# wahn/rs_pbrt

Measured on NVIDIA H100. Metric: Mrays/s, higher is better.
Workload: dtype f32

## Files before the change

### rs_pbrt_b200/csrc/pb_kernels.cuh

```cuda
#pragma once
#include "pb_bsdf.cuh"
#include "pb_interaction.cuh"
#include "pb_sobol.cuh"
#include "pb_texture.cuh"
#include "pb_material.cuh"

namespace pb {

#define PB_TRACE_THREADS 128
#define PB_TRACE_SMEM_BYTES 49152
#define PB_SHADE_THREADS 128
#define PB_SMEM_SOBOL_BYTES 49152

#ifdef PB_HOST_EMU
PB_D void mbar_init(uint64_t*, uint32_t) {}
PB_D void mbar_fence_init() {}
PB_D void mbar_expect_tx(uint64_t*, uint32_t) {}
PB_D void tma_bulk_g2s(void* dst_smem, const void* src_gmem, uint32_t bytes, uint64_t*) { memcpy(dst_smem, src_gmem, bytes); }
PB_D void mbar_wait(uint64_t*, uint32_t) { __syncthreads(); }
#define PB_DYNAMIC_SMEM(name) unsigned char* name = emu::g_dyn_smem
#else
#define PB_DYNAMIC_SMEM(name) extern __shared__ __align__(16) unsigned char name[]
PB_D void mbar_fence_init() { asm volatile("fence.mbarrier_init.release.cluster;" ::: "memory"); }
PB_D uint32_t smem_u32(const void* p) { return (uint32_t)__cvta_generic_to_shared(p); }
// ... 315 lines not shown
    float4* o = wide + 4 * (size_t)i;
    o[0] = make_float4(a[0].x, a[0].y, a[0].z, a[0].w);
    o[1] = make_float4(b[0].x, b[0].y, a[1].x, a[1].y);
    o[2] = make_float4(a[1].z, a[1].w, b[1].x, b[1].y);
    o[3] = make_float4(__uint_as_float(ref[0]), __uint_as_float(ref[1]), __uint_as_float((meta >> 16) & 3u), 0.0f);
}
#ifndef PB_WIDE_MIN_BLOCKS
#define PB_WIDE_MIN_BLOCKS 0
#endif
#ifndef PB_WIDE_INST_MIN_BLOCKS
#define PB_WIDE_INST_MIN_BLOCKS 8
#endif
#if PB_WIDE_MIN_BLOCKS > 0
#define PB_WIDE_BOUNDS __launch_bounds__(PB_TRACE_THREADS, PB_WIDE_MIN_BLOCKS)
#else
#define PB_WIDE_BOUNDS __launch_bounds__(PB_TRACE_THREADS)
#endif
__global__ void PB_WIDE_BOUNDS k_trace_wide_plain(DScene sc, TraceIO io, const uint32_t* __restrict__ d_nrays, uint32_t* __restrict__ cursor, DCounters* cnt, int walk_steps) {
    trace_rays_wide<false>(sc, sc.wide, sc.tri_verts, io, *d_nrays, cursor, cnt, walk_steps);
}
__global__ void __launch_bounds__(PB_TRACE_THREADS, PB_WIDE_INST_MIN_BLOCKS) k_trace_wide_inst(DScene sc, TraceIO io, const uint32_t* __restrict__ d_nrays, uint32_t* __restrict__ cursor,
                                                                                             DCounters* cnt, int walk_steps) {
    trace_rays_wide<true>(sc, sc.wide, sc.tri_verts, io, *d_nrays, cursor, cnt, walk_steps);
}

__global__ void PB_WIDE_BOUNDS k_trace_wide_spec(DScene sc, TraceIO io, const uint32_t* __restrict__ d_nrays,
                                                                                        uint32_t* __restrict__ cursor, DCounters* cnt, int walk_steps) {
    trace_rays_wide_spec(sc, sc.wide, sc.tri_verts, io, *d_nrays, cursor, cnt, walk_steps);
}

__global__ void __launch_bounds__(256) k_rayprep(const float4* __restrict__ rays, const uint32_t* __restrict__ d_nrays, float4* __restrict__ pre) {
    const uint32_t n = *d_nrays;
    for (uint32_t i = blockIdx.x * blockDim.x + threadIdx.x; i < n; i += gridDim.x * blockDim.x) {
        const float4 a = rays[2 * (size_t)i], b = rays[2 * (size_t)i + 1];
        const RayPre r = make_ray(mk3(a.x, a.y, a.z), mk3(b.x, b.y, b.z));
        float4 p0, p1;
        pack_ray(r, p0, p1);
        pre[2 * (size_t)i] = p0;
        pre[2 * (size_t)i + 1] = p1;
    }
}

__global__ void __launch_bounds__(256) k_sort(DScene sc, DPaths ps, DLightGrid grid, uint32_t spatial, uint32_t instancing, const uint32_t* __restrict__ queue,
                                             const uint32_t* __restrict__ d_count, uint32_t* __restrict__ cls_queue, uint32_t cls_stride,
                                             uint32_t* __restrict__ cls_count, uint32_t* __restrict__ reset_count_out, uint32_t* __restrict__ reset_nrays) {
    if (blockIdx.x == 0 && threadIdx.x == 0) { *reset_count_out = 0u; *reset_nrays = 0u; }
    const uint32_t count = *d_count;
    const uint32_t lane = threadIdx.x & 31;
    const uint32_t total = (count + 31u) & ~31u;
    for (uint32_t qi = blockIdx.x * blockDim.x + threadIdx.x; qi < total; qi += gridDim.x * blockDim.x) {
        uint32_t cls = 0xffffffffu, slot = 0;
        if (qi < count) {
            slot = queue[qi];
            cls = 0;
            if (__float_as_uint(ps.L[slot].w) & PF_HAS_RAY) {
                float4 h = ps.hit[slot];
                int prim = __float_as_int(h.x);
                if (prim >= 0) {
                    float4 c = __ldg(sc.tri_verts + 3 * (size_t)prim + 2);
                    uint32_t mat = __float_as_uint(c.y);
                    const uint32_t inst = sc.n_instances ? ps.hit_inst[slot] : 0xffffffffu;
                    const bool moved = inst != 0xffffffffu && !sc.instances[inst].identity;
                    if (moved && instancing == 0u) mat = 0xffffffffu;
                    cls = (mat == 0xffffffffu) ? 1u : ((uint32_t)sc.materials[mat].cls & 0xffu);
                    if (spatial) {
                        float4 a = __ldg(sc.tri_verts + 3 * (size_t)prim), b = __ldg(sc.tri_verts + 3 * (size_t)prim + 1);
                        V3 p = mk3(a.x, a.y, a.z) * h.y + mk3(a.w, b.x, b.y) * h.z + mk3(b.z, b.w, c.x) * h.w;
                        if (moved) {
                            const float* m = sc.instances[inst].m;
                            const float xp = m[0] * p.x + m[1] * p.y + m[2] * p.z + m[3], yp = m[4] * p.x + m[5] * p.y + m[6] * p.z + m[7];
                            const float zp = m[8] * p.x + m[9] * p.y + m[10] * p.z + m[11], wp = m[12] * p.x + m[13] * p.y + m[14] * p.z + m[15];
                            p = mk3(xp, yp, zp);
                            if (wp != 1.0f) { const float inv = 1.0f / wp; p = mk3(inv * xp, inv * yp, inv * zp); }
                        }
                        uint32_t v = light_voxel(sc, grid, p);
                        if (grid.state[v] == 0 && atomicCAS(&grid.state[v], 0, 1) == 0) {
                            if (grid.row) {
                                uint32_t r = atomicAdd(grid.n_request + 1, 1u);
                                if (r >= grid.max_rows) { r = 0u; atomicOr(grid.n_request + 2, 1u); }
                                grid.row[v] = (int)r;
                            }
                            grid.request[atomicAdd(grid.n_request, 1u)] = v;
                        }
                    }
                }
            }
        }
        unsigned peers = __match_any_sync(0xffffffffu, cls);
        uint32_t base = 0;
        int leader = __ffs(peers) - 1;
        if (cls != 0xffffffffu && (int)lane == leader) base = atomicAdd(cls_count + cls, (uint32_t)__popc(peers));
        base = __shfl_sync(0xffffffffu, base, leader);
        if (cls != 0xffffffffu) cls_queue[(size_t)cls * cls_stride + base + (uint32_t)__popc(peers & ((1u << lane) - 1u))] = slot;
    }
}

__global__ void k_lightgrid_contrib(DScene sc, DLightGrid g, const float* __restrict__ halton ) {
    uint32_t nreq = *g.n_request;
    uint32_t total = nreq * (uint32_t)g.n_lights;
    for (uint32_t i = blockIdx.x * blockDim.x + threadIdx.x; i < total; i += gridDim.x * blockDim.x) {
        uint32_t v = g.request[i / (uint32_t)g.n_lights], j = i % (uint32_t)g.n_lights;
        int ix = (int)(v % (uint32_t)g.nv[0]), iy = (int)((v / (uint32_t)g.nv[0]) % (uint32_t)g.nv[1]), iz = (int)(v / ((uint32_t)g.nv[0] * (uint32_t)g.nv[1]));
        float t0x = (float)ix / (float)g.nv[0], t0y = (float)iy / (float)g.nv[1], t0z = (float)iz / (float)g.nv[2];
        float t1x = (float)(ix + 1) / (float)g.nv[0], t1y = (float)(iy + 1) / (float)g.nv[1], t1z = (float)(iz + 1) / (float)g.nv[2];
        V3 vmin = mk3(lerpf(t0x, sc.wb_min[0], sc.wb_max[0]), lerpf(t0y, sc.wb_min[1], sc.wb_max[1]), lerpf(t0z, sc.wb_min[2], sc.wb_max[2]));
        V3 vmax = mk3(lerpf(t1x, sc.wb_min[0], sc.wb_max[0]), lerpf(t1y, sc.wb_min[1], sc.wb_max[1]), lerpf(t1z, sc.wb_min[2], sc.wb_max[2]));
        const DLight& light = sc.lights[j];
        float contrib = 0.0f;
        for (int s = 0; s < 128; ++s) {
            const float* hs = halton + 5 * s;
            V3 po = mk3(lerpf(__ldg(hs), vmin.x, vmax.x), lerpf(__ldg(hs + 1), vmin.y, vmax.y), lerpf(__ldg(hs + 2), vmin.z, vmax.z));
            float pdf = 0.0f;
            V3 wi;
            LightSample ls;
            Sp li = light_sample_li<false>(sc, light, po, make_float2(__ldg(hs + 3), __ldg(hs + 4)), wi, pdf, ls);
            if (pdf > 0.0f) contrib += lum(li) / pdf;
        }
        g.contrib[g.row_of(v) * g.n_lights + j] = contrib;
    }
}
__global__ void k_lightgrid_build(DLightGrid g) {
    uint32_t nreq = *g.n_request;
    const int nl = g.n_lights;
    for (uint32_t i = blockIdx.x * blockDim.x + threadIdx.x; i < nreq; i += gridDim.x * blockDim.x) {
        uint32_t v = g.request[i];
        const size_t r = g.row_of(v);
        const float* c = g.contrib + r * nl;
        float sum = 0.0f;
        for (int j = 0; j < nl; ++j) sum += c[j];
        float avg = sum / (float)(128 * nl);
        float min_contrib = (avg > 0.0f) ? 0.001f * avg : 1.0f;
        float* func = g.func + r * nl;
        float* cdf = g.cdf + r * (nl + 1);
        cdf[0] = 0.0f;
        for (int j = 0; j < nl; ++j) {
            float f = fmaxf(c[j], min_contrib);
            func[j] = f;
            cdf[j + 1] = cdf[j] + f / (float)nl;
        }
// ... 219 lines not shown
    PB_DYNAMIC_SMEM(smem_raw);
    __shared__ __align__(8) uint64_t s_bar;
    if (blockIdx.x == 0 && threadIdx.x < PB_SHADE_CLASSES) {
        reset_cls_count[threadIdx.x] = 0u;
        if (threadIdx.x == 0) { *reset_cursor = 0u; if (reset_requests) *reset_requests = 0u; }
    }
    const uint32_t* tab = nib;
    const uint32_t tab_stride = sobol_cfg & 0xffffu;
    if (!HALTON && (sobol_cfg >> 31)) {
        const uint32_t bytes = n_chunks * 64u * tab_stride;
        if (threadIdx.x == 0) {
            mbar_init(&s_bar, 1);
            mbar_fence_init();
        }
        __syncthreads();
        if (threadIdx.x == 0) {
            mbar_expect_tx(&s_bar, bytes);
            for (uint32_t off = 0; off < bytes; off += 16384u)
                tma_bulk_g2s(smem_raw + off, reinterpret_cast<const unsigned char*>(nib) + off, min(16384u, bytes - off), &s_bar);
        }
        mbar_wait(&s_bar, 0);
        tab = reinterpret_cast<const uint32_t*>(smem_raw);
    }
    __shared__ uint32_t s_tiles[PB_SHADE_CLASSES + 1];
    if (threadIdx.x == 0) {
        uint32_t acc = 0;
        for (uint32_t c = 0; c < PB_SHADE_CLASSES; ++c) { s_tiles[c] = acc; if (c >= cls_lo && c < cls_hi) acc += (cls_count[c] + 31u) >> 5; }
        s_tiles[PB_SHADE_CLASSES] = acc;
    }
    __syncthreads();
    const uint32_t total_tiles = s_tiles[PB_SHADE_CLASSES];
    const int NONSPEC = BSDF_ALL & ~BSDF_SPECULAR;
    const float inf = __int_as_float(0x7f800000);
    uint32_t n_light_tests = 0, n_slots = 0, n_vertices = 0;
    const uint32_t warps_total = (gridDim.x * blockDim.x) >> 5;
    const uint32_t warp_id = (blockIdx.x * blockDim.x + threadIdx.x) >> 5;
    const uint32_t lane = threadIdx.x & 31;
    for (uint32_t tile = warp_id; tile < total_tiles; tile += warps_total) {
        uint32_t cls = 0;
        while (cls + 1 < PB_SHADE_CLASSES && tile >= s_tiles[cls + 1]) ++cls;
        const uint32_t qi = (tile - s_tiles[cls]) * 32u + lane;
        const uint32_t count = cls_count[cls];
        bool push = false, emit_ext = false, emit_sh = false, emit_mis = false;
        float4 ext0, ext1, sh0, sh1, mis0, mis1;
        ext0 = ext1 = sh0 = sh1 = mis0 = mis1 = make_float4(0.0f, 0.0f, 0.0f, 0.0f);
        uint32_t slot = 0;
        if (qi < count) {
            slot = cls_queue[(size_t)cls * cls_stride + qi];
            n_slots++;
            const float4 Lf = ps.L[slot];
            const float4 st_hit = ps.hit[slot], st_rd = ps.ray_d[slot], st_beta = ps.beta[slot];
            const uint2 st_sobol = ps.sobol[slot];
            const uint32_t st_dim = ps.dim[slot];
            const float4 st_ld = ps.ld_light[slot], st_mh = ps.mis_hit[slot], st_md = ps.mis_d[slot], st_mf = ps.mis_f[slot], st_nb = ps.nee_beta[slot];
            const uint32_t st_occl = ps.occl[slot];
            uint32_t flags = __float_as_uint(Lf.w);
            Sp L = mksp(Lf.x, Lf.y, Lf.z);
            if (flags & (PF_HAS_SHADOW | PF_HAS_MIS)) {
                Sp ld = sp1(0.0f);
                const float4 a = st_ld;
                if ((flags & PF_HAS_SHADOW) && st_occl == 0u) ld = ld + mksp(a.x, a.y, a.z);
                if (flags & PF_HAS_MIS) {
                    const float4 mh = st_mh;
                    int mprim = __float_as_int(mh.x);
                    if (mprim >= 0) {
                        const float4 md = st_md, mf = st_mf;
                        int light_num = (int)__float_as_uint(md.w);
                        V3 lp, ln;
                        int hit_light;
                        tri_point_normal(sc, (uint32_t)mprim, mh.y, mh.z, mh.w, lp, ln, hit_light);
                        if (hit_light == light_num) {
                            Sp le = light_L(sc.lights[light_num], ln, -mk3(md.x, md.y, md.z));
                            if (!is_black(le)) ld = ld + mksp(mf.x, mf.y, mf.z) * le * sp1(1.0f) * a.w / mf.w;
                        }
                    } else if (!AREA_ONLY && sc.n_inf) {
                        const float4 md = st_md, mf = st_mf;
                        Sp le = light_le(sc, sc.lights[__float_as_uint(md.w)], mk3(md.x, md.y, md.z));
                        if (!is_black(le)) ld = ld + mksp(mf.x, mf.y, mf.z) * le * sp1(1.0f) * a.w / mf.w;
                    }
                }
                const float4 nb = st_nb;
                L = L + mksp(nb.x, nb.y, nb.z) * spdiv0(ld, nb.w);
            }
            uint32_t out_flags = 0;
            if (!AREA_ONLY && cls == 0u && sc.n_inf && (flags & PF_HAS_RAY) && __float_as_int(st_hit.x) < 0) {
                if ((flags >> PF_BOUNCES_SHIFT) == 0 || (flags & PF_SPECULAR_BOUNCE)) {
                    const Sp beta = mksp(st_beta.x, st_beta.y, st_beta.z);
                    const V3 rd = mk3(st_rd.x, st_rd.y, st_rd.z);
                    for (uint32_t k = 0; k < sc.n_inf; ++k) L = L + beta * light_le(sc, sc.lights[sc.inf[k]], rd);
                }
            }
            if (cls != 0u) {
                uint32_t bounces = flags >> PF_BOUNCES_SHIFT;
                bool specular_bounce = (flags & PF_SPECULAR_BOUNCE) != 0;
                const float4 hit = st_hit;
                int prim = __float_as_int(hit.x);
                if (prim >= 0) {
                    n_vertices++;
                    const float4 rd4 = st_rd, b4 = st_beta;
                    V3 rd = mk3(rd4.x, rd4.y, rd4.z);
                    Sp beta = mksp(b4.x, b4.y, b4.z);
                    float eta_scale = b4.w;
                    V3 wo = -rd;
                    V3 wo_nee = wo;
                    Isect is = INST ? hit_interaction(sc, rp.instancing, (uint32_t)prim, hit.y, hit.z, hit.w, ps.hit_inst[slot], rd, wo_nee)
                                              : tri_interaction(sc, (uint32_t)prim, hit.y, hit.z, hit.w);
                    if (bounces == 0 || specular_bounce) {
                        const Sp le = is.area_light >= 0 ? light_L(sc.lights[is.area_light], is.n, wo) : sp1(0.0f);
                        L = L + beta * le;
                    }
                    if (bounces < rp.max_depth) {
                        if (is.material == 0xffffffffu) {
                            V3 o = offset_ray_origin(is.p, is.p_error, is.n, rd);
                            ext0 = make_float4(o.x, o.y, o.z, inf);
                            ext1 = make_float4(rd.x, rd.y, rd.z, __uint_as_float(slot | (RAY_EXTEND << 30)));
                            emit_ext = true;
                            out_flags = (flags & ~0xffu) | (flags & PF_SPECULAR_BOUNCE) | PF_HAS_RAY;
                        } else {
                            BsdfFrame B;
                            B.mat = sc.materials + is.material;
                            if (SPEC == 0 && (B.mat->cls & PB_MAT_TEXTURED)) {
                                if (B.mat->cls & PB_MAT_BUMPED) {
                                    const float4 f0 = ps.slot_frame[2 * (size_t)slot], f1 = ps.slot_frame[2 * (size_t)slot + 1];
                                    is.ns = mk3(f0.x, f0.y, f0.z);
                                    is.sh_dpdu = mk3(f1.x, f1.y, f1.z);
                                }
                                B.mat = ps.slot_mat + slot;
                            }
                            B.ns = is.ns;
                            B.ng = is.n;
                            B.ss = norm3(is.sh_dpdu);
                            B.ts = cross3(is.ns, B.ss);
                            const uint2 si = st_sobol;
                            SobolT sob;
                            sob.nib = tab;
                            sob.ds = tab_stride;
                            sob.n_chunks = n_chunks;
                            sob.index = ((uint64_t)si.y << 32) | si.x;
                            sob.dim = st_dim;
                            sob.overflow = false;
                            uint32_t nee_flags = 0;
                            if (SPEC >= 1 ? pb_spec_has_nonspecular(SPEC) : (B.mat->nonspecular > 0)) {
                                Sp ld_now = sp1(0.0f);
                                const int nl = grid.n_lights;
                                if (nl > 0) {
                                    const size_t v = (rp.light_strategy == 2u) ? grid.row_of(light_voxel(sc, grid, is.p)) : (size_t)0;
                                    float choice_pdf;
                                    float u5[5];
                                    if (HALTON) {
#pragma unroll
                                        for (int k = 0; k < 5; ++k) u5[k] = halton_scrambled(rp, (uint32_t)sob.index, min(sob.dim + (uint32_t)k, (uint32_t)(PB_HALTON_DIMS - 1)));
                                    } else sobolT_fill<5>(sob, u5);
                                    const float u_choice = sobolT_take<HALTON>(sob, 1) ? u5[0] : 0.0f;
                                    int light_num = sample_discrete(grid.func + v * nl, grid.cdf + v * (nl + 1), grid.func_int[v], nl,
                                                                    u_choice, choice_pdf);
                                    if (choice_pdf != 0.0f) {
                                        float2 u_light = make_float2(0.0f, 0.0f), u_scat = make_float2(0.0f, 0.0f);
                                        if (sobolT_take<HALTON>(sob, 2)) u_light = make_float2(u5[1], u5[2]);
                                        if (sobolT_take<HALTON>(sob, 2)) u_scat = make_float2(u5[3], u5[4]);
                                        const DLight& light = sc.lights[light_num];
                                        V3 wi = mk3(0.0f, 0.0f, 0.0f);
                                        float light_pdf = 0.0f, scattering_pdf = 0.0f, mis_w = 0.0f;
                                        Sp a = sp1(0.0f);
                                        LightSample ls;
                                        Sp li = light_sample_li<AREA_ONLY>(sc, light, is.p, u_light, wi, light_pdf, ls);
                                        if (light_pdf > 0.0f && !is_black(li)) {
                                            Sp f = bsdf_f<SPEC>(B, wo_nee, wi, NONSPEC) * sp1(absdot3(wi, is.ns));
                                            scattering_pdf = bsdf_pdf<SPEC>(B, wo_nee, wi, NONSPEC);
                                            if (!is_black(f)) {
                                                V3 origin = offset_ray_origin(is.p, is.p_error, is.n, ls.p - is.p);
                                                V3 target = offset_ray_origin(ls.p, ls.p_error, ls.n, origin - ls.p);
                                                V3 sd = target - origin;
                                                if (!AREA_ONLY && light_is_delta(light)) a = f * li / light_pdf;
                                                else {
                                                    float w = power_heuristic(light_pdf, scattering_pdf);
                                                    a = f * li * sp1(w) / light_pdf;
                                                }
                                                sh0 = make_float4(origin.x, origin.y, origin.z, 1.0f - PB_SHADOW_EPSILON);
                                                sh1 = make_float4(sd.x, sd.y, sd.z, __uint_as_float(slot | (RAY_SHADOW << 30)));
                                                emit_sh = true;
                                                nee_flags |= PF_HAS_SHADOW;
                                            }
                                        }
                                        int st = 0;
                                        Sp f2 = sp1(0.0f);
                                        if (AREA_ONLY || !light_is_delta(light)) {
                                            f2 = bsdf_sample_f<SPEC>(B, wo_nee, wi, u_scat, scattering_pdf, NONSPEC, st);
                                            f2 = f2 * sp1(absdot3(wi, is.ns));
                                        }
                                        if (!is_black(f2) && scattering_pdf > 0.0f) {
                                            V3 mo = offset_ray_origin(is.p, is.p_error, is.n, wi);
                                            if (AREA_ONLY || light.kind == 0u) n_light_tests++;
                                            float lp = light_pdf_li<AREA_ONLY>(sc, light, is.p, mo, wi);
                                            if (lp != 0.0f) {
                                                mis_w = power_heuristic(scattering_pdf, lp);
                                                mis0 = make_float4(mo.x, mo.y, mo.z, inf);
                                                mis1 = make_float4(wi.x, wi.y, wi.z, __uint_as_float(slot | (RAY_MIS << 30)));
                                                emit_mis = true;
                                                ps.mis_d[slot] = make_float4(wi.x, wi.y, wi.z, __uint_as_float((uint32_t)light_num));
                                                ps.mis_f[slot] = make_float4(f2.r, f2.g, f2.b, scattering_pdf);
                                                nee_flags |= PF_HAS_MIS;
                                            }
                                        }
                                        if (nee_flags) {
                                            ps.ld_light[slot] = make_float4(a.r, a.g, a.b, mis_w);
                                            ps.nee_beta[slot] = make_float4(beta.r, beta.g, beta.b, choice_pdf);
                                        } else ld_now = spdiv0(sp1(0.0f), choice_pdf);
                                    }
                                }
                                if (!nee_flags) L = L + beta * ld_now;
                            }
                            V3 wi = mk3(0.0f, 0.0f, 0.0f);
                            float pdf = 0.0f;
                            int st = 255;
                            float u3[3];
                            if (HALTON) {
                                u3[0] = halton_scrambled(rp, (uint32_t)sob.index, min(sob.dim, (uint32_t)(PB_HALTON_DIMS - 1)));
                                u3[1] = halton_scrambled(rp, (uint32_t)sob.index, min(sob.dim + 1u, (uint32_t)(PB_HALTON_DIMS - 1)));
                                u3[2] = 0.0f;
                            } else sobolT_fill<3>(sob, u3);
                            const float2 u_bsdf = sobolT_take<HALTON>(sob, 2) ? make_float2(u3[0], u3[1]) : make_float2(0.0f, 0.0f);
                            Sp f = bsdf_sample_f<SPEC>(B, wo, wi, u_bsdf, pdf, BSDF_ALL, st);
                            bool alive = !(is_black(f) || pdf == 0.0f);
                            if (alive) {
                                beta = beta * ((f * absdot3(wi, is.ns)) / pdf);
                                specular_bounce = (st & BSDF_SPECULAR) != 0;
                                if ((st & BSDF_SPECULAR) && (st & BSDF_TRANSMISSION)) {
                                    float eta = B.mat->eta;
                                    if (dot3(wo, is.n) > 0.0f) eta_scale *= eta * eta;
                                    else eta_scale *= 1.0f / (eta * eta);
                                }
                                V3 o = offset_ray_origin(is.p, is.p_error, is.n, wi);
                                Sp rr_beta = beta * eta_scale;
                                if (maxsp(rr_beta) < rp.rr_threshold && bounces > 3) {
                                    float q = fmaxf(0.05f, 1.0f - maxsp(rr_beta));
                                    if (HALTON) u3[2] = halton_scrambled(rp, (uint32_t)sob.index, min(sob.dim, (uint32_t)(PB_HALTON_DIMS - 1)));
                                    const float u_rr = sobolT_take<HALTON>(sob, 1) ? u3[2] : 0.0f;
                                    if (u_rr < q) alive = false;
                                    else beta = beta / (1.0f - q);
                                }
                                if (alive) {
                                    ext0 = make_float4(o.x, o.y, o.z, inf);
                                    ext1 = make_float4(wi.x, wi.y, wi.z, __uint_as_float(slot | (RAY_EXTEND << 30)));
                                    emit_ext = true;
                                    ps.ray_d[slot] = make_float4(wi.x, wi.y, wi.z, 0.0f);
                                    ps.beta[slot] = make_float4(beta.r, beta.g, beta.b, eta_scale);
                                    ps.dim[slot] = sob.dim;
                                    out_flags = ((bounces + 1) << PF_BOUNCES_SHIFT) | (specular_bounce ? PF_SPECULAR_BOUNCE : 0u) | PF_HAS_RAY;
                                }
                            }
                            out_flags |= nee_flags;
                            if (sob.overflow) atomicOr(d_error, 1u);
                        }
                    }
                }
            }
            ps.L[slot] = make_float4(L.r, L.g, L.b, __uint_as_float(out_flags));
            push = (out_flags & (PF_HAS_RAY | PF_HAS_SHADOW | PF_HAS_MIS)) != 0;
        }
        const unsigned mp = __ballot_sync(0xffffffffu, push);
        const unsigned me = __ballot_sync(0xffffffffu, emit_ext), mm = __ballot_sync(0xffffffffu, emit_mis), ms = __ballot_sync(0xffffffffu, emit_sh);
        const uint32_t ne = (uint32_t)__popc(me), nm = (uint32_t)__popc(mm), nsh = (uint32_t)__popc(ms);
        uint32_t qbase = 0, rbase = 0;
        if (lane == 0) {
            if (mp) qbase = atomicAdd(d_count_out, (uint32_t)__popc(mp));
            if (ne + nm + nsh) rbase = atomicAdd(d_nrays, ne + nm + nsh);
        }
        qbase = __shfl_sync(0xffffffffu, qbase, 0);
        rbase = __shfl_sync(0xffffffffu, rbase, 0);
        if (push) queue_out[qbase + (uint32_t)__popc(mp & ((1u << lane) - 1u))] = slot;
        const unsigned lt = (1u << lane) - 1u;
        if (emit_ext) { size_t q = rbase + (uint32_t)__popc(me & lt); rays[2 * q] = ext0; rays[2 * q + 1] = ext1; if (ray_keys) ray_keys[q] = ray_key(sc, ext0, ext1) & key_mask; }
        if (emit_mis) { size_t q = rbase + ne + (uint32_t)__popc(mm & lt); rays[2 * q] = mis0; rays[2 * q + 1] = mis1; if (ray_keys) ray_keys[q] = ray_key(sc, mis0, mis1) & key_mask; }
        if (emit_sh) { size_t q = rbase + ne + nm + (uint32_t)__popc(ms & lt); rays[2 * q] = sh0; rays[2 * q + 1] = sh1; if (ray_keys) ray_keys[q] = ray_key(sc, sh0, sh1) & key_mask; }
    }
    uint32_t t = warp_sum(n_light_tests);
    if (lane == 0 && t) atomicAdd(&cnt->light_tri_tests, (unsigned long long)t);
    t = warp_sum(n_slots);
    if (lane == 0 && t) atomicAdd(&cnt->shade_slots, (unsigned long long)t);
    t = warp_sum(n_vertices);
    if (lane == 0 && t) atomicAdd(&cnt->shaded_vertices, (unsigned long long)t);
}

PB_D V3 uniform_sample_hemisphere(float2 u) {
    float z = u.x;
    float r = sqrtf(fmaxf(0.0f, 1.0f - z * z));
    float phi = 2.0f * PB_PI * u.y;
    float sp, cp;
    sincos_rn(phi, sp, cp);
    return mk3(r * cp, r * sp, z);
}
__global__ void __launch_bounds__(256) k_ao_shade(DScene sc, DRender rp, DPaths ps, BatchInfo bi, uint32_t ao_n, uint32_t ao_cos, const uint32_t* __restrict__ nib,
                                                  uint32_t n_chunks, const uint64_t* __restrict__ vdc, const uint64_t* __restrict__ vdci,
                                                  float4* __restrict__ rays, float* __restrict__ weight, uint32_t* __restrict__ d_nrays) {
    __shared__ uint64_t s_vdc[52], s_vdci[52];
    if (threadIdx.x < 52) {
        uint32_t m = rp.log2_res;
        s_vdc[threadIdx.x] = m ? vdc[(m - 1) * 52 + threadIdx.x] : 0;
        s_vdci[threadIdx.x] = m ? vdci[(m - 1) * 52 + threadIdx.x] : 0;
    }
    __syncthreads();
    const uint32_t n_paths = bi.n_pixels * bi.n_samples;
    const uint64_t total = (uint64_t)n_paths * ao_n;
    const uint64_t gid = (uint64_t)blockIdx.x * blockDim.x + threadIdx.x;
    float4 r0 = make_float4(0.0f, 0.0f, 0.0f, 0.0f), r1 = r0;
    bool live = false;
    if (gid < total) {
// ... 141 lines not shown
```

### rs_pbrt_b200/csrc/pbrt_gpu.cu

```cuda
#include <sched.h>

#include <algorithm>
#include <chrono>
#include <cmath>
#include <cstdio>
#include <cstdlib>
#include <atomic>
#include <cstring>
#include <functional>
#include <map>
#include <memory>
#include <mutex>
#include <string>
#include <thread>
#include <vector>

#include "../../include/pbrt_gpu.h"
#include "pb_kernels.cuh"
#include "pb_direct.cuh"

using namespace pb;

extern "C" {
extern const unsigned char pb_sobol_blob_start[];
// ... 1576 lines not shown
                int rc = trace();
                if (rc != PBRT_OK) return rc;
                CK(cudaMemsetAsync(d_nrays, 0, 4, st));
                cudaEvent_t e, f;
                CK(scr->event(&e)); CK(scr->event(&f));
                CK(cudaEventRecord(e, st));
                const uint64_t total = (uint64_t)n * ao_n;
                k_ao_shade<<<(unsigned)((total + 255) / 256), 256, 0, st>>>(sc->d, rp, ps, bi, ao_n, p->ao_cos_sample ? 1u : 0u, sc->nib.p, n_chunks, sc->vdc.p,
                                                                         sc->vdci.p, X.rays.p, X.ao_weight.p, d_nrays);
                CK(cudaEventRecord(f, st));
                sev.push_back(e); sev.push_back(f);
                launches++;
                if ((rc = trace()) != PBRT_OK) return rc;
                k_ao_resolve<<<(n + 255) / 256, 256, 0, st>>>(ps, bi, ao_n, X.ao_weight.p, X.occl.p);
                k_resolve<<<(bi.n_pixels + 255) / 256, 256, 0, st>>>(rp, ps, bi, scr->filter_table.p, d_film, d_samples);
                launches += 2;
            }
        CK(cudaGetLastError());
        CK(cudaEventRecord(ev1, st));
        CK(cudaStreamSynchronize(st));
    } else if (share_pixels > 0) {
        const uint64_t total_pixels = share_pixels;
        static const int cap_log2_env = getenv("PB_BATCH_LOG2") ? std::min(26, std::max(10, atoi(getenv("PB_BATCH_LOG2")))) : 0;
        const int cap_log2 = cap_log2_env ? cap_log2_env : (sc->d.n_textures ? 22 : 24);
        const size_t CAP = (size_t)1 << cap_log2;
        const uint32_t samples_per_batch = (uint32_t)std::min<size_t>(rp.spp, CAP);
        const uint32_t pixels_per_batch = (uint32_t)std::min<uint64_t>(std::max<size_t>(1, CAP / samples_per_batch), total_pixels);
        const size_t cap = (size_t)samples_per_batch * pixels_per_batch;
        const uint64_t n_batches = ((rp.spp + samples_per_batch - 1) / samples_per_batch) * ((total_pixels + pixels_per_batch - 1) / pixels_per_batch);
        static const int shade_spec = getenv("PB_SHADE_SPEC") ? atoi(getenv("PB_SHADE_SPEC")) : 2;
        const bool plan_instanced = sc->d.n_instances > 0;
        struct ShadeLaunch { int spec; uint32_t lo, hi; };
        std::vector<ShadeLaunch> shade_plan;
        {
            uint32_t mask = sc->class_mask & ~1u, covered = 0;
            const uint32_t first_general = PB_SPEC_PLASTIC + 1;
            for (uint32_t c = 1; c < first_general && shade_spec; ++c) {
                if (!(mask & (1u << c))) continue;
                const bool have = c == 1 + LOBE_LAMBERT || (shade_spec >= 2 && !halton && !plan_instanced && (c == 1 + LOBE_SPEC_REFL || c == 1 + LOBE_FRESNEL_SPEC || c == 1 + LOBE_OREN_NAYAR ||
                                                                                                    c == 1 + LOBE_MF_REFL || c == 1 + LOBE_FRESNEL_BLEND || c == PB_SPEC_PLASTIC));
                if (!have) continue;
                shade_plan.push_back({(int)c, c, c + 1});
                covered |= 1u << c;
            }
            const uint32_t rest = mask & ~covered;
            for (uint32_t c = 1; c < PB_SHADE_CLASSES;) {
                if (!(rest & (1u << c))) { ++c; continue; }
                uint32_t e = c;
                while (e < PB_SHADE_CLASSES && (rest & (1u << e))) ++e;
                shade_plan.push_back({0, c, e});
                c = e;
            }
            const uint32_t lam = 1 + LOBE_LAMBERT;
            bool folded = false;
            if ((covered & (1u << lam)) && (mask & ((1u << lam) - 2u)) == 0u)
                for (ShadeLaunch& l : shade_plan) if (l.spec == (int)lam) { l.lo = 0; folded = true; }
            if (!folded) shade_plan.insert(shade_plan.begin(), ShadeLaunch{shade_spec ? (int)lam : 0, 0u, (mask & 2u) ? 1u : 2u});
        }
        static const bool dual_env = !(getenv("PB_SINGLE_STREAM") && atoi(getenv("PB_SINGLE_STREAM")));
        const bool streams_forced = getenv("PB_STREAMS") && atoi(getenv("PB_STREAMS")) >= 2;
        const bool dual = dual_env && !(p->flags & PBRT_RENDER_SINGLE_STREAM) && !null_paths && n_batches > 1 &&
                          !(getenv("PB_STREAMS") && atoi(getenv("PB_STREAMS")) <= 1) && ((shade_plan.size() >= 3 && sc->d.n_textures == 0) || streams_forced);
        static const int streams_env = getenv("PB_STREAMS") ? std::min(4, std::max(1, atoi(getenv("PB_STREAMS")))) : 2;
        const int n_ctx = dual ? (int)std::min<uint64_t>((uint64_t)streams_env, n_batches) : 1;

        const int sm_count = sm_count_of(sc->device);
        const bool count_work = (p->flags & PBRT_RENDER_COUNT_WORK) != 0;
        const bool spatial = strategy == PBRT_LIGHTS_SPATIAL && nl > 0;

        int nv[3] = {1, 1, 1};
        size_t nvox = 1;
        if (spatial) {
            float diag[3] = {sc->d.wb_max[0] - sc->d.wb_min[0], sc->d.wb_max[1] - sc->d.wb_min[1], sc->d.wb_max[2] - sc->d.wb_min[2]};
            int me = (diag[0] > diag[1] && diag[0] > diag[2]) ? 0 : (diag[1] > diag[2] ? 1 : 2);
            float bmax = diag[me];
            for (int i = 0; i < 3; ++i) {
                nv[i] = std::max(1, f2i_sat(roundf(diag[i] / bmax * 64.0f)));
                nvox *= (size_t)nv[i];
            }
        }
        const size_t grid_row_bytes = (3 * std::max<size_t>(nl, 1) + 2) * sizeof(float);
        const size_t grid_budget = lightgrid_budget();
        const bool grid_sparse = spatial && nvox * grid_row_bytes > grid_budget;
        const size_t grid_rows = grid_sparse ? std::max<size_t>(1, std::min(nvox, grid_budget / grid_row_bytes)) : nvox;
        std::vector<float> fixed_f(nl, 1.0f), fixed_cdf;
        float fixed_int = 0.0f;
        if (!spatial && nl > 0) {
            if (strategy == PBRT_LIGHTS_POWER)
                for (uint32_t j = 0; j < nl; ++j) {
                    const DLight& l = sc->h_lights[j];
                    Sp pw;
                    const Sp I = mksp(l.L[0], l.L[1], l.L[2]);
                    if (l.kind == PBRT_LIGHT_POINT) pw = I * (4.0f * PB_PI);
                    else if (l.kind == PBRT_LIGHT_SPOT) pw = I * 2.0f * PB_PI * (1.0f - 0.5f * (l.cos_falloff_start + l.cos_total_width));
                    else if (l.kind == PBRT_LIGHT_DISTANT) pw = I * PB_PI * sc->d.world_radius * sc->d.world_radius;
                    else if (l.kind == PBRT_LIGHT_INFINITE) pw = sc->h_env_power[j] * sp1(PB_PI * sc->d.world_radius * sc->d.world_radius);
                    else pw = I * (l.two_sided ? 2.0f : 1.0f) * l.area * PB_PI;
                    fixed_f[j] = lum(pw);
                }
            make_distribution(fixed_f, fixed_cdf, fixed_int);
        }
        CK(scr->filter_table.alloc(256));
        CK(cudaMemcpyAsync(scr->filter_table.p, p->filter_table, 256 * 4, cudaMemcpyHostToDevice, st));

        uint32_t dims_needed = (uint32_t)std::min<uint64_t>(1024u, 5 + 8 * ((uint64_t)rp.max_depth + 1));
        uint32_t log2_spp = 0;
        while ((1u << log2_spp) < rp.spp) log2_spp++;
        const uint32_t index_bits = std::min<uint32_t>(52u, 2u * rp.log2_res + log2_spp);
        const uint32_t n_chunks = std::max<uint32_t>(1u, (index_bits + 3u) / 4u);
        const uint32_t sobol_ds = (dims_needed + 8u) | 1u;
// ... 635 lines not shown
```

Measured before the change: 1513.

## Resolve deferred NEE/MIS and env misses in sort kernel, drop class-0 shading

Moves the accumulation of deferred shadow/MIS contributions and the environment-light handling for missed rays out of the shade kernel into the sort kernel, which already reads each path's L. Finished paths (class 0) are now retired directly in sort, so shading launches no longer have to cover class 0. The host shade plan is changed so that class 0 is never launched and class 1 is launched only when needed. The sort kernel gains extra loads and light evaluation, which may raise its register pressure and divergence.

```diff
diff --git a/rs_pbrt_b200/csrc/pb_kernels.cuh b/rs_pbrt_b200/csrc/pb_kernels.cuh
--- a/rs_pbrt_b200/csrc/pb_kernels.cuh
+++ b/rs_pbrt_b200/csrc/pb_kernels.cuh
@@ -391,11 +391,46 @@
         uint32_t cls = 0xffffffffu, slot = 0;
         if (qi < count) {
             slot = queue[qi];
-            cls = 0;
-            if (__float_as_uint(ps.L[slot].w) & PF_HAS_RAY) {
+            const float4 Lf = ps.L[slot];
+            const uint32_t flags = __float_as_uint(Lf.w);
+            Sp L = mksp(Lf.x, Lf.y, Lf.z);
+            if (flags & (PF_HAS_SHADOW | PF_HAS_MIS)) {
+                Sp ld = sp1(0.0f);
+                const float4 a = ps.ld_light[slot];
+                if ((flags & PF_HAS_SHADOW) && ps.occl[slot] == 0u) ld = ld + mksp(a.x, a.y, a.z);
+                if (flags & PF_HAS_MIS) {
+                    const float4 mh = ps.mis_hit[slot];
+                    int mprim = __float_as_int(mh.x);
+                    if (mprim >= 0) {
+                        const float4 md = ps.mis_d[slot], mf = ps.mis_f[slot];
+                        int light_num = (int)__float_as_uint(md.w);
+                        V3 lp, ln;
+                        int hit_light;
+                        tri_point_normal(sc, (uint32_t)mprim, mh.y, mh.z, mh.w, lp, ln, hit_light);
+                        if (hit_light == light_num) {
+                            Sp le = light_L(sc.lights[light_num], ln, -mk3(md.x, md.y, md.z));
+                            if (!is_black(le)) ld = ld + mksp(mf.x, mf.y, mf.z) * le * sp1(1.0f) * a.w / mf.w;
+                        }
+                    } else if (sc.n_inf) {
+                        const float4 md = ps.mis_d[slot], mf = ps.mis_f[slot];
+                        Sp le = light_le(sc, sc.lights[__float_as_uint(md.w)], mk3(md.x, md.y, md.z));
+                        if (!is_black(le)) ld = ld + mksp(mf.x, mf.y, mf.z) * le * sp1(1.0f) * a.w / mf.w;
+                    }
+                }
+                const float4 nb = ps.nee_beta[slot];
+                L = L + mksp(nb.x, nb.y, nb.z) * spdiv0(ld, nb.w);
+            }
+            if (flags & PF_HAS_RAY) {
                 float4 h = ps.hit[slot];
                 int prim = __float_as_int(h.x);
-                if (prim >= 0) {
+                if (prim < 0) {
+                    if (sc.n_inf && ((flags >> PF_BOUNCES_SHIFT) == 0 || (flags & PF_SPECULAR_BOUNCE))) {
+                        const float4 b4 = ps.beta[slot], rd4 = ps.ray_d[slot];
+                        const Sp beta = mksp(b4.x, b4.y, b4.z);
+                        const V3 rd = mk3(rd4.x, rd4.y, rd4.z);
+                        for (uint32_t k = 0; k < sc.n_inf; ++k) L = L + beta * light_le(sc, sc.lights[sc.inf[k]], rd);
+                    }
+                } else {
                     float4 c = __ldg(sc.tri_verts + 3 * (size_t)prim + 2);
                     uint32_t mat = __float_as_uint(c.y);
                     const uint32_t inst = sc.n_instances ? ps.hit_inst[slot] : 0xffffffffu;
@@ -424,6 +459,8 @@
                     }
                 }
             }
+            if (cls == 0xffffffffu) ps.L[slot] = make_float4(L.r, L.g, L.b, __uint_as_float(0u));
+            else if (flags & (PF_HAS_SHADOW | PF_HAS_MIS)) ps.L[slot] = make_float4(L.r, L.g, L.b, __uint_as_float(flags & ~(PF_HAS_SHADOW | PF_HAS_MIS)));
         }
         unsigned peers = __match_any_sync(0xffffffffu, cls);
         uint32_t base = 0;
@@ -749,207 +786,168 @@
             const float4 st_hit = ps.hit[slot], st_rd = ps.ray_d[slot], st_beta = ps.beta[slot];
             const uint2 st_sobol = ps.sobol[slot];
             const uint32_t st_dim = ps.dim[slot];
-            const float4 st_ld = ps.ld_light[slot], st_mh = ps.mis_hit[slot], st_md = ps.mis_d[slot], st_mf = ps.mis_f[slot], st_nb = ps.nee_beta[slot];
-            const uint32_t st_occl = ps.occl[slot];
             uint32_t flags = __float_as_uint(Lf.w);
             Sp L = mksp(Lf.x, Lf.y, Lf.z);
-            if (flags & (PF_HAS_SHADOW | PF_HAS_MIS)) {
-                Sp ld = sp1(0.0f);
-                const float4 a = st_ld;
-                if ((flags & PF_HAS_SHADOW) && st_occl == 0u) ld = ld + mksp(a.x, a.y, a.z);
-                if (flags & PF_HAS_MIS) {
-                    const float4 mh = st_mh;
-                    int mprim = __float_as_int(mh.x);
-                    if (mprim >= 0) {
-                        const float4 md = st_md, mf = st_mf;
-                        int light_num = (int)__float_as_uint(md.w);
-                        V3 lp, ln;
-                        int hit_light;
-                        tri_point_normal(sc, (uint32_t)mprim, mh.y, mh.z, mh.w, lp, ln, hit_light);
-                        if (hit_light == light_num) {
-                            Sp le = light_L(sc.lights[light_num], ln, -mk3(md.x, md.y, md.z));
-                            if (!is_black(le)) ld = ld + mksp(mf.x, mf.y, mf.z) * le * sp1(1.0f) * a.w / mf.w;
+            uint32_t out_flags = 0;
+            uint32_t bounces = flags >> PF_BOUNCES_SHIFT;
+            bool specular_bounce = (flags & PF_SPECULAR_BOUNCE) != 0;
+            const float4 hit = st_hit;
+            int prim = __float_as_int(hit.x);
+            n_vertices++;
+            const float4 rd4 = st_rd, b4 = st_beta;
+            V3 rd = mk3(rd4.x, rd4.y, rd4.z);
+            Sp beta = mksp(b4.x, b4.y, b4.z);
+            float eta_scale = b4.w;
+            V3 wo = -rd;
+            V3 wo_nee = wo;
+            Isect is = INST ? hit_interaction(sc, rp.instancing, (uint32_t)prim, hit.y, hit.z, hit.w, ps.hit_inst[slot], rd, wo_nee)
+                                      : tri_interaction(sc, (uint32_t)prim, hit.y, hit.z, hit.w);
+            if (bounces == 0 || specular_bounce) {
+                const Sp le = is.area_light >= 0 ? light_L(sc.lights[is.area_light], is.n, wo) : sp1(0.0f);
+                L = L + beta * le;
+            }
+            if (bounces < rp.max_depth) {
+                if (is.material == 0xffffffffu) {
+                    V3 o = offset_ray_origin(is.p, is.p_error, is.n, rd);
+                    ext0 = make_float4(o.x, o.y, o.z, inf);
+                    ext1 = make_float4(rd.x, rd.y, rd.z, __uint_as_float(slot | (RAY_EXTEND << 30)));
+                    emit_ext = true;
+                    out_flags = (flags & ~0xffu) | (flags & PF_SPECULAR_BOUNCE) | PF_HAS_RAY;
+                } else {
+                    BsdfFrame B;
+                    B.mat = sc.materials + is.material;
+                    if (SPEC == 0 && (B.mat->cls & PB_MAT_TEXTURED)) {
+                        if (B.mat->cls & PB_MAT_BUMPED) {
+                            const float4 f0 = ps.slot_frame[2 * (size_t)slot], f1 = ps.slot_frame[2 * (size_t)slot + 1];
+                            is.ns = mk3(f0.x, f0.y, f0.z);
+                            is.sh_dpdu = mk3(f1.x, f1.y, f1.z);
                         }
-                    } else if (!AREA_ONLY && sc.n_inf) {
-                        const float4 md = st_md, mf = st_mf;
-                        Sp le = light_le(sc, sc.lights[__float_as_uint(md.w)], mk3(md.x, md.y, md.z));
-                        if (!is_black(le)) ld = ld + mksp(mf.x, mf.y, mf.z) * le * sp1(1.0f) * a.w / mf.w;
+                        B.mat = ps.slot_mat + slot;
                     }
-                }
-                const float4 nb = st_nb;
-                L = L + mksp(nb.x, nb.y, nb.z) * spdiv0(ld, nb.w);
-            }
-            uint32_t out_flags = 0;
-            if (!AREA_ONLY && cls == 0u && sc.n_inf && (flags & PF_HAS_RAY) && __float_as_int(st_hit.x) < 0) {
-                if ((flags >> PF_BOUNCES_SHIFT) == 0 || (flags & PF_SPECULAR_BOUNCE)) {
-                    const Sp beta = mksp(st_beta.x, st_beta.y, st_beta.z);
-                    const V3 rd = mk3(st_rd.x, st_rd.y, st_rd.z);
-                    for (uint32_t k = 0; k < sc.n_inf; ++k) L = L + beta * light_le(sc, sc.lights[sc.inf[k]], rd);
-                }
-            }
-            if (cls != 0u) {
-                uint32_t bounces = flags >> PF_BOUNCES_SHIFT;
-                bool specular_bounce = (flags & PF_SPECULAR_BOUNCE) != 0;
-                const float4 hit = st_hit;
-                int prim = __float_as_int(hit.x);
-                if (prim >= 0) {
-                    n_vertices++;
-                    const float4 rd4 = st_rd, b4 = st_beta;
-                    V3 rd = mk3(rd4.x, rd4.y, rd4.z);
-                    Sp beta = mksp(b4.x, b4.y, b4.z);
-                    float eta_scale = b4.w;
-                    V3 wo = -rd;
-                    V3 wo_nee = wo;
-                    Isect is = INST ? hit_interaction(sc, rp.instancing, (uint32_t)prim, hit.y, hit.z, hit.w, ps.hit_inst[slot], rd, wo_nee)
-                                              : tri_interaction(sc, (uint32_t)prim, hit.y, hit.z, hit.w);
-                    if (bounces == 0 || specular_bounce) {
-                        const Sp le = is.area_light >= 0 ? light_L(sc.lights[is.area_light], is.n, wo) : sp1(0.0f);
-                        L = L + beta * le;
-                    }
-                    if (bounces < rp.max_depth) {
-                        if (is.material == 0xffffffffu) {
-                            V3 o = offset_ray_origin(is.p, is.p_error, is.n, rd);
-                            ext0 = make_float4(o.x, o.y, o.z, inf);
-                            ext1 = make_float4(rd.x, rd.y, rd.z, __uint_as_float(slot | (RAY_EXTEND << 30)));
-                            emit_ext = true;
-                            out_flags = (flags & ~0xffu) | (flags & PF_SPECULAR_BOUNCE) | PF_HAS_RAY;
-                        } else {
-                            BsdfFrame B;
-                            B.mat = sc.materials + is.material;
-                            if (SPEC == 0 && (B.mat->cls & PB_MAT_TEXTURED)) {
-                                if (B.mat->cls & PB_MAT_BUMPED) {
-                                    const float4 f0 = ps.slot_frame[2 * (size_t)slot], f1 = ps.slot_frame[2 * (size_t)slot + 1];
-                                    is.ns = mk3(f0.x, f0.y, f0.z);
-                                    is.sh_dpdu = mk3(f1.x, f1.y, f1.z);
-                                }
-                                B.mat = ps.slot_mat + slot;
-                            }
-                            B.ns = is.ns;
-                            B.ng = is.n;
-                            B.ss = norm3(is.sh_dpdu);
-                            B.ts = cross3(is.ns, B.ss);
-                            const uint2 si = st_sobol;
-                            SobolT sob;
-                            sob.nib = tab;
-                            sob.ds = tab_stride;
-                            sob.n_chunks = n_chunks;
-                            sob.index = ((uint64_t)si.y << 32) | si.x;
-                            sob.dim = st_dim;
-                            sob.overflow = false;
-                            uint32_t nee_flags = 0;
-                            if (SPEC >= 1 ? pb_spec_has_nonspecular(SPEC) : (B.mat->nonspecular > 0)) {
-                                Sp ld_now = sp1(0.0f);
-                                const int nl = grid.n_lights;
-                                if (nl > 0) {
-                                    const size_t v = (rp.light_strategy == 2u) ? grid.row_of(light_voxel(sc, grid, is.p)) : (size_t)0;
-                                    float choice_pdf;
-                                    float u5[5];
-                                    if (HALTON) {
+                    B.ns = is.ns;
+                    B.ng = is.n;
+                    B.ss = norm3(is.sh_dpdu);
+                    B.ts = cross3(is.ns, B.ss);
+                    const uint2 si = st_sobol;
+                    SobolT sob;
+                    sob.nib = tab;
+                    sob.ds = tab_stride;
+                    sob.n_chunks = n_chunks;
+                    sob.index = ((uint64_t)si.y << 32) | si.x;
+                    sob.dim = st_dim;
+                    sob.overflow = false;
+                    uint32_t nee_flags = 0;
+                    if (SPEC >= 1 ? pb_spec_has_nonspecular(SPEC) : (B.mat->nonspecular > 0)) {
+                        Sp ld_now = sp1(0.0f);
+                        const int nl = grid.n_lights;
+                        if (nl > 0) {
+                            const size_t v = (rp.light_strategy == 2u) ? grid.row_of(light_voxel(sc, grid, is.p)) : (size_t)0;
+                            float choice_pdf;
+                            float u5[5];
+                            if (HALTON) {
 #pragma unroll
-                                        for (int k = 0; k < 5; ++k) u5[k] = halton_scrambled(rp, (uint32_t)sob.index, min(sob.dim + (uint32_t)k, (uint32_t)(PB_HALTON_DIMS - 1)));
-                                    } else sobolT_fill<5>(sob, u5);
-                                    const float u_choice = sobolT_take<HALTON>(sob, 1) ? u5[0] : 0.0f;
-                                    int light_num = sample_discrete(grid.func + v * nl, grid.cdf + v * (nl + 1), grid.func_int[v], nl,
-                                                                    u_choice, choice_pdf);
-                                    if (choice_pdf != 0.0f) {
-                                        float2 u_light = make_float2(0.0f, 0.0f), u_scat = make_float2(0.0f, 0.0f);
-                                        if (sobolT_take<HALTON>(sob, 2)) u_light = make_float2(u5[1], u5[2]);
-                                        if (sobolT_take<HALTON>(sob, 2)) u_scat = make_float2(u5[3], u5[4]);
-                                        const DLight& light = sc.lights[light_num];
-                                        V3 wi = mk3(0.0f, 0.0f, 0.0f);
-                                        float light_pdf = 0.0f, scattering_pdf = 0.0f, mis_w = 0.0f;
-                                        Sp a = sp1(0.0f);
-                                        LightSample ls;
-                                        Sp li = light_sample_li<AREA_ONLY>(sc, light, is.p, u_light, wi, light_pdf, ls);
-                                        if (light_pdf > 0.0f && !is_black(li)) {
-                                            Sp f = bsdf_f<SPEC>(B, wo_nee, wi, NONSPEC) * sp1(absdot3(wi, is.ns));
-                                            scattering_pdf = bsdf_pdf<SPEC>(B, wo_nee, wi, NONSPEC);
-                                            if (!is_black(f)) {
-                                                V3 origin = offset_ray_origin(is.p, is.p_error, is.n, ls.p - is.p);
-                                                V3 target = offset_ray_origin(ls.p, ls.p_error, ls.n, origin - ls.p);
-                                                V3 sd = target - origin;
-                                                if (!AREA_ONLY && light_is_delta(light)) a = f * li / light_pdf;
-                                                else {
-                                                    float w = power_heuristic(light_pdf, scattering_pdf);
-                                                    a = f * li * sp1(w) / light_pdf;
-                                                }
-                                                sh0 = make_float4(origin.x, origin.y, origin.z, 1.0f - PB_SHADOW_EPSILON);
-                                                sh1 = make_float4(sd.x, sd.y, sd.z, __uint_as_float(slot | (RAY_SHADOW << 30)));
-                                                emit_sh = true;
-                                                nee_flags |= PF_HAS_SHADOW;
-                                            }
+                                for (int k = 0; k < 5; ++k) u5[k] = halton_scrambled(rp, (uint32_t)sob.index, min(sob.dim + (uint32_t)k, (uint32_t)(PB_HALTON_DIMS - 1)));
+                            } else sobolT_fill<5>(sob, u5);
+                            const float u_choice = sobolT_take<HALTON>(sob, 1) ? u5[0] : 0.0f;
+                            int light_num = sample_discrete(grid.func + v * nl, grid.cdf + v * (nl + 1), grid.func_int[v], nl,
+                                                            u_choice, choice_pdf);
+                            if (choice_pdf != 0.0f) {
+                                float2 u_light = make_float2(0.0f, 0.0f), u_scat = make_float2(0.0f, 0.0f);
+                                if (sobolT_take<HALTON>(sob, 2)) u_light = make_float2(u5[1], u5[2]);
+                                if (sobolT_take<HALTON>(sob, 2)) u_scat = make_float2(u5[3], u5[4]);
+                                const DLight& light = sc.lights[light_num];
+                                V3 wi = mk3(0.0f, 0.0f, 0.0f);
+                                float light_pdf = 0.0f, scattering_pdf = 0.0f, mis_w = 0.0f;
+                                Sp a = sp1(0.0f);
+                                LightSample ls;
+                                Sp li = light_sample_li<AREA_ONLY>(sc, light, is.p, u_light, wi, light_pdf, ls);
+                                if (light_pdf > 0.0f && !is_black(li)) {
+                                    Sp f = bsdf_f<SPEC>(B, wo_nee, wi, NONSPEC) * sp1(absdot3(wi, is.ns));
+                                    scattering_pdf = bsdf_pdf<SPEC>(B, wo_nee, wi, NONSPEC);
+                                    if (!is_black(f)) {
+                                        V3 origin = offset_ray_origin(is.p, is.p_error, is.n, ls.p - is.p);
+                                        V3 target = offset_ray_origin(ls.p, ls.p_error, ls.n, origin - ls.p);
+                                        V3 sd = target - origin;
+                                        if (!AREA_ONLY && light_is_delta(light)) a = f * li / light_pdf;
+                                        else {
+                                            float w = power_heuristic(light_pdf, scattering_pdf);
+                                            a = f * li * sp1(w) / light_pdf;
                                         }
-                                        int st = 0;
-                                        Sp f2 = sp1(0.0f);
-                                        if (AREA_ONLY || !light_is_delta(light)) {
-                                            f2 = bsdf_sample_f<SPEC>(B, wo_nee, wi, u_scat, scattering_pdf, NONSPEC, st);
-                                            f2 = f2 * sp1(absdot3(wi, is.ns));
-                                        }
-                                        if (!is_black(f2) && scattering_pdf > 0.0f) {
-                                            V3 mo = offset_ray_origin(is.p, is.p_error, is.n, wi);
-                                            if (AREA_ONLY || light.kind == 0u) n_light_tests++;
-                                            float lp = light_pdf_li<AREA_ONLY>(sc, light, is.p, mo, wi);
-                                            if (lp != 0.0f) {
-                                                mis_w = power_heuristic(scattering_pdf, lp);
-                                                mis0 = make_float4(mo.x, mo.y, mo.z, inf);
-                                                mis1 = make_float4(wi.x, wi.y, wi.z, __uint_as_float(slot | (RAY_MIS << 30)));
-                                                emit_mis = true;
-                                                ps.mis_d[slot] = make_float4(wi.x, wi.y, wi.z, __uint_as_float((uint32_t)light_num));
-                                                ps.mis_f[slot] = make_float4(f2.r, f2.g, f2.b, scattering_pdf);
-                                                nee_flags |= PF_HAS_MIS;
-                                            }
-                                        }
-                                        if (nee_flags) {
-                                            ps.ld_light[slot] = make_float4(a.r, a.g, a.b, mis_w);
-                                            ps.nee_beta[slot] = make_float4(beta.r, beta.g, beta.b, choice_pdf);
-                                        } else ld_now = spdiv0(sp1(0.0f), choice_pdf);
+                                        sh0 = make_float4(origin.x, origin.y, origin.z, 1.0f - PB_SHADOW_EPSILON);
+                                        sh1 = make_float4(sd.x, sd.y, sd.z, __uint_as_float(slot | (RAY_SHADOW << 30)));
+                                        emit_sh = true;
+                                        nee_flags |= PF_HAS_SHADOW;
                                     }
                                 }
-                                if (!nee_flags) L = L + beta * ld_now;
+                                int st = 0;
+                                Sp f2 = sp1(0.0f);
+                                if (AREA_ONLY || !light_is_delta(light)) {
+                                    f2 = bsdf_sample_f<SPEC>(B, wo_nee, wi, u_scat, scattering_pdf, NONSPEC, st);
+                                    f2 = f2 * sp1(absdot3(wi, is.ns));
+                                }
+                                if (!is_black(f2) && scattering_pdf > 0.0f) {
+                                    V3 mo = offset_ray_origin(is.p, is.p_error, is.n, wi);
+                                    if (AREA_ONLY || light.kind == 0u) n_light_tests++;
+                                    float lp = light_pdf_li<AREA_ONLY>(sc, light, is.p, mo, wi);
+                                    if (lp != 0.0f) {
+                                        mis_w = power_heuristic(scattering_pdf, lp);
+                                        mis0 = make_float4(mo.x, mo.y, mo.z, inf);
+                                        mis1 = make_float4(wi.x, wi.y, wi.z, __uint_as_float(slot | (RAY_MIS << 30)));
+                                        emit_mis = true;
+                                        ps.mis_d[slot] = make_float4(wi.x, wi.y, wi.z, __uint_as_float((uint32_t)light_num));
+                                        ps.mis_f[slot] = make_float4(f2.r, f2.g, f2.b, scattering_pdf);
+                                        nee_flags |= PF_HAS_MIS;
+                                    }
+                                }
+                                if (nee_flags) {
+                                    ps.ld_light[slot] = make_float4(a.r, a.g, a.b, mis_w);
+                                    ps.nee_beta[slot] = make_float4(beta.r, beta.g, beta.b, choice_pdf);
+                                } else ld_now = spdiv0(sp1(0.0f), choice_pdf);
                             }
-                            V3 wi = mk3(0.0f, 0.0f, 0.0f);
-                            float pdf = 0.0f;
-                            int st = 255;
-                            float u3[3];
-                            if (HALTON) {
-                                u3[0] = halton_scrambled(rp, (uint32_t)sob.index, min(sob.dim, (uint32_t)(PB_HALTON_DIMS - 1)));
-                                u3[1] = halton_scrambled(rp, (uint32_t)sob.index, min(sob.dim + 1u, (uint32_t)(PB_HALTON_DIMS - 1)));
-                                u3[2] = 0.0f;
-                            } else sobolT_fill<3>(sob, u3);
-                            const float2 u_bsdf = sobolT_take<HALTON>(sob, 2) ? make_float2(u3[0], u3[1]) : make_float2(0.0f, 0.0f);
-                            Sp f = bsdf_sample_f<SPEC>(B, wo, wi, u_bsdf, pdf, BSDF_ALL, st);
-                            bool alive = !(is_black(f) || pdf == 0.0f);
-                            if (alive) {
-                                beta = beta * ((f * absdot3(wi, is.ns)) / pdf);
-                                specular_bounce = (st & BSDF_SPECULAR) != 0;
-                                if ((st & BSDF_SPECULAR) && (st & BSDF_TRANSMISSION)) {
-                                    float eta = B.mat->eta;
-                                    if (dot3(wo, is.n) > 0.0f) eta_scale *= eta * eta;
-                                    else eta_scale *= 1.0f / (eta * eta);
-                                }
-                                V3 o = offset_ray_origin(is.p, is.p_error, is.n, wi);
-                                Sp rr_beta = beta * eta_scale;
-                                if (maxsp(rr_beta) < rp.rr_threshold && bounces > 3) {
-                                    float q = fmaxf(0.05f, 1.0f - maxsp(rr_beta));
-                                    if (HALTON) u3[2] = halton_scrambled(rp, (uint32_t)sob.index, min(sob.dim, (uint32_t)(PB_HALTON_DIMS - 1)));
-                                    const float u_rr = sobolT_take<HALTON>(sob, 1) ? u3[2] : 0.0f;
-                                    if (u_rr < q) alive = false;
-                                    else beta = beta / (1.0f - q);
-                                }
-                                if (alive) {
-                                    ext0 = make_float4(o.x, o.y, o.z, inf);
-                                    ext1 = make_float4(wi.x, wi.y, wi.z, __uint_as_float(slot | (RAY_EXTEND << 30)));
-                                    emit_ext = true;
-                                    ps.ray_d[slot] = make_float4(wi.x, wi.y, wi.z, 0.0f);
-                                    ps.beta[slot] = make_float4(beta.r, beta.g, beta.b, eta_scale);
-                                    ps.dim[slot] = sob.dim;
-                                    out_flags = ((bounces + 1) << PF_BOUNCES_SHIFT) | (specular_bounce ? PF_SPECULAR_BOUNCE : 0u) | PF_HAS_RAY;
-                                }
-                            }
-                            out_flags |= nee_flags;
-                            if (sob.overflow) atomicOr(d_error, 1u);
+                        }
+                        if (!nee_flags) L = L + beta * ld_now;
+                    }
+                    V3 wi = mk3(0.0f, 0.0f, 0.0f);
+                    float pdf = 0.0f;
+                    int st = 255;
+                    float u3[3];
+                    if (HALTON) {
+                        u3[0] = halton_scrambled(rp, (uint32_t)sob.index, min(sob.dim, (uint32_t)(PB_HALTON_DIMS - 1)));
+                        u3[1] = halton_scrambled(rp, (uint32_t)sob.index, min(sob.dim + 1u, (uint32_t)(PB_HALTON_DIMS - 1)));
+                        u3[2] = 0.0f;
+                    } else sobolT_fill<3>(sob, u3);
+                    const float2 u_bsdf = sobolT_take<HALTON>(sob, 2) ? make_float2(u3[0], u3[1]) : make_float2(0.0f, 0.0f);
+                    Sp f = bsdf_sample_f<SPEC>(B, wo, wi, u_bsdf, pdf, BSDF_ALL, st);
+                    bool alive = !(is_black(f) || pdf == 0.0f);
+                    if (alive) {
+                        beta = beta * ((f * absdot3(wi, is.ns)) / pdf);
+                        specular_bounce = (st & BSDF_SPECULAR) != 0;
+                        if ((st & BSDF_SPECULAR) && (st & BSDF_TRANSMISSION)) {
+                            float eta = B.mat->eta;
+                            if (dot3(wo, is.n) > 0.0f) eta_scale *= eta * eta;
+                            else eta_scale *= 1.0f / (eta * eta);
+                        }
+                        V3 o = offset_ray_origin(is.p, is.p_error, is.n, wi);
+                        Sp rr_beta = beta * eta_scale;
+                        if (maxsp(rr_beta) < rp.rr_threshold && bounces > 3) {
+                            float q = fmaxf(0.05f, 1.0f - maxsp(rr_beta));
+                            if (HALTON) u3[2] = halton_scrambled(rp, (uint32_t)sob.index, min(sob.dim, (uint32_t)(PB_HALTON_DIMS - 1)));
+                            const float u_rr = sobolT_take<HALTON>(sob, 1) ? u3[2] : 0.0f;
+                            if (u_rr < q) alive = false;
+                            else beta = beta / (1.0f - q);
+                        }
+                        if (alive) {
+                            ext0 = make_float4(o.x, o.y, o.z, inf);
+                            ext1 = make_float4(wi.x, wi.y, wi.z, __uint_as_float(slot | (RAY_EXTEND << 30)));
+                            emit_ext = true;
+                            ps.ray_d[slot] = make_float4(wi.x, wi.y, wi.z, 0.0f);
+                            ps.beta[slot] = make_float4(beta.r, beta.g, beta.b, eta_scale);
+                            ps.dim[slot] = sob.dim;
+                            out_flags = ((bounces + 1) << PF_BOUNCES_SHIFT) | (specular_bounce ? PF_SPECULAR_BOUNCE : 0u) | PF_HAS_RAY;
                         }
                     }
+                    out_flags |= nee_flags;
+                    if (sob.overflow) atomicOr(d_error, 1u);
                 }
             }
             ps.L[slot] = make_float4(L.r, L.g, L.b, __uint_as_float(out_flags));
diff --git a/rs_pbrt_b200/csrc/pbrt_gpu.cu b/rs_pbrt_b200/csrc/pbrt_gpu.cu
--- a/rs_pbrt_b200/csrc/pbrt_gpu.cu
+++ b/rs_pbrt_b200/csrc/pbrt_gpu.cu
@@ -1652,10 +1652,13 @@
                 c = e;
             }
             const uint32_t lam = 1 + LOBE_LAMBERT;
-            bool folded = false;
-            if ((covered & (1u << lam)) && (mask & ((1u << lam) - 2u)) == 0u)
-                for (ShadeLaunch& l : shade_plan) if (l.spec == (int)lam) { l.lo = 0; folded = true; }
-            if (!folded) shade_plan.insert(shade_plan.begin(), ShadeLaunch{shade_spec ? (int)lam : 0, 0u, (mask & 2u) ? 1u : 2u});
+            const bool null_hits = sc->has_null_material || (plan_instanced && p->instancing == PBRT_INSTANCING_REFERENCE);
+            if (!(mask & 2u) && (null_hits || shade_plan.empty())) {
+                bool folded = false;
+                if ((covered & (1u << lam)) && (mask & ((1u << lam) - 4u)) == 0u)
+                    for (ShadeLaunch& l : shade_plan) if (l.spec == (int)lam) { l.lo = 1; folded = true; }
+                if (!folded) shade_plan.insert(shade_plan.begin(), ShadeLaunch{shade_spec ? (int)lam : 0, 1u, 2u});
+            }
         }
         static const bool dual_env = !(getenv("PB_SINGLE_STREAM") && atoi(getenv("PB_SINGLE_STREAM")));
         const bool streams_forced = getenv("PB_STREAMS") && atoi(getenv("PB_STREAMS")) >= 2;
```

Measured after the change: 1588, median of 6. 5.0% higher.
